# microsoft/rl-offline-simulation

Measured on AMD Instinct MI355X. Metric: simulated steps/sec (node), 10M logged transitions x 4096 rollouts, higher is better.
Workload: dtype f64

## Files before the change

### rl-offline-simulation_amd/csrc/offsim_hip.hip

```cpp
#include <hip/hip_fp16.h>
#include <hip/hip_runtime.h>
#include <mutex>
#include <stdint.h>
#include <stdio.h>
#include <stdlib.h>
#include <string.h>
#include <time.h>

#include "offsim.h"
#include "discount.hpp"
#include "pcg64_dev.hpp"
#include "philox_dev.hpp"

extern "C" int offsim_lds_order_ok(void);
#include "shuffle_wave.hpp"
#include "shuffle_chunk.hpp"

using namespace offsim;

static thread_local char g_err[512] = "";

static int fail(int code, const char *fmt, const char *detail = "") {
    snprintf(g_err, sizeof(g_err), fmt, detail);
    return code;
// ... 62 lines not shown
        if (s < n_slots) seg_off[s] = carry + inc - v;
        carry += __shfl(inc, WAVE - 1);
    }
    if (lane == 0) seg_off[n_slots] = carry;
}
__global__ void k_group_scatter(const int32_t *__restrict__ slot, int64_t N, int32_t n_slots,
                                const uint32_t *__restrict__ hist, const uint32_t *__restrict__ seg_off,
                                int32_t *__restrict__ order) {
    extern __shared__ uint32_t lds_pos_raw[];
    volatile uint32_t *lds_pos = lds_pos_raw;
    const uint32_t *h = hist + (int64_t)blockIdx.x * n_slots;
    for (int s = threadIdx.x; s < n_slots; s += WAVE) lds_pos[s] = seg_off[s] + h[s];
    __syncthreads();
    int lane = threadIdx.x;
    int64_t base = (int64_t)blockIdx.x * GRP_CHUNK;
    for (int i = 0; i < GRP_CHUNK; i += WAVE) {
        int64_t row = base + i + lane;
        bool valid = row < N;
        int32_t key = valid ? slot[row] : -1;
        uint64_t todo = __ballot(valid);
        uint32_t dst = 0;
        while (todo) {
            int leader = __ffsll((unsigned long long)todo) - 1;
            int32_t k = __shfl(key, leader);
            uint64_t same = __ballot(valid && key == k);
            if (valid && key == k) {
                uint32_t before = __popcll(same & ((1ull << lane) - 1ull));
                dst = lds_pos[k] + before;
            }
            __builtin_amdgcn_s_waitcnt(0xc07f);
            if (lane == leader) lds_pos[k] += __popcll(same);
            todo &= ~same;
        }
        if (valid) order[dst] = (int32_t)row;
    }
}

extern "C" int64_t offsim_group_scratch_bytes(int64_t N, int32_t n_slots) {
    int64_t n_chunks = (N + GRP_CHUNK - 1) / GRP_CHUNK;
    if (n_chunks < 1) n_chunks = 1;
    return (n_chunks * n_slots + n_slots) * (int64_t)sizeof(uint32_t) + 256;
}

extern "C" int offsim_group_by_state(const int32_t *slot, int64_t N, int32_t n_slots, uint32_t *seg_off, int32_t *order,
                                     void *scratch, void *stream) {
    if (N < 0 || n_slots <= 0 || !seg_off || !scratch) return fail(OFFSIM_EINVAL, "group_by_state: bad argument%s");
    if ((int64_t)n_slots * 4 > 64 * 1024) return fail(OFFSIM_EUNSUPPORTED, "group_by_state: more than 16384 states%s");
    if (N >= (1ll << 31)) return fail(OFFSIM_EUNSUPPORTED, "group_by_state: N >= 2^31%s");
    hipStream_t st = (hipStream_t)stream;
    int64_t n_chunks = (N + GRP_CHUNK - 1) / GRP_CHUNK;
    uint32_t *hist = (uint32_t *)scratch;
    uint32_t *totals = hist + (n_chunks > 0 ? n_chunks : 1) * n_slots;
    if (n_chunks == 0) {
        HIP_TRY(hipMemsetAsync(seg_off, 0, sizeof(uint32_t) * (n_slots + 1), st));
        return OFFSIM_OK;
    }
    size_t lds = sizeof(uint32_t) * n_slots;
    hipLaunchKernelGGL(k_group_hist, dim3((unsigned)n_chunks), dim3(256), lds, st, slot, N, n_slots, hist);
    LAUNCH_CHECK();
    hipLaunchKernelGGL(k_group_scan_chunks, dim3((n_slots + 63) / 64), dim3(64), 0, st, hist, n_chunks, n_slots, totals);
    LAUNCH_CHECK();
    hipLaunchKernelGGL(k_group_scan_slots, dim3(1), dim3(WAVE), 0, st, totals, n_slots, seg_off);
    LAUNCH_CHECK();
    hipLaunchKernelGGL(k_group_scatter, dim3((unsigned)n_chunks), dim3(WAVE), lds, st, slot, N, n_slots, hist, seg_off, order);
    LAUNCH_CHECK();
    return OFFSIM_OK;
}

template <typename T>
__global__ void k_gather_elem(const T *__restrict__ src, const int32_t *__restrict__ order, int64_t N, T *__restrict__ dst) {
    int64_t g = (int64_t)blockIdx.x * blockDim.x + threadIdx.x;
    if (g < N) dst[g] = src[order[g]];
}
template <typename W>
__global__ void k_gather_words(const W *__restrict__ src, const int32_t *__restrict__ order, int64_t N, int32_t words, W *__restrict__ dst) {
    int64_t i = (int64_t)blockIdx.x * blockDim.x + threadIdx.x;
    if (i >= N * words) return;
    int64_t g = i / words;
    int32_t w = (int32_t)(i - g * words);
    dst[i] = src[(int64_t)order[g] * words + w];
}
extern "C" int offsim_gather_rows(const void *src, const int32_t *order, int64_t N, int32_t row_bytes, void *dst, void *stream) {
    if (N < 0 || row_bytes <= 0) return fail(OFFSIM_EINVAL, "gather_rows: bad argument%s");
    if (N == 0) return OFFSIM_OK;
    hipStream_t st = (hipStream_t)stream;
    unsigned nb = (unsigned)((N + 255) / 256);
    if (row_bytes == 1) hipLaunchKernelGGL(k_gather_elem<uint8_t>, dim3(nb), dim3(256), 0, st, (const uint8_t *)src, order, N, (uint8_t *)dst);
    else if (row_bytes == 2) hipLaunchKernelGGL(k_gather_elem<uint16_t>, dim3(nb), dim3(256), 0, st, (const uint16_t *)src, order, N, (uint16_t *)dst);
    else if (row_bytes == 4) hipLaunchKernelGGL(k_gather_elem<uint32_t>, dim3(nb), dim3(256), 0, st, (const uint32_t *)src, order, N, (uint32_t *)dst);
    else if (row_bytes == 8) hipLaunchKernelGGL(k_gather_elem<uint64_t>, dim3(nb), dim3(256), 0, st, (const uint64_t *)src, order, N, (uint64_t *)dst);
    else {
        const int32_t wb = row_bytes % 4 == 0 ? 4 : row_bytes % 2 == 0 ? 2 : 1, words = row_bytes / wb;
        unsigned nbw = (unsigned)((N * words + 255) / 256);
        if (wb == 4) hipLaunchKernelGGL(k_gather_words<uint32_t>, dim3(nbw), dim3(256), 0, st, (const uint32_t *)src, order, N, words, (uint32_t *)dst);
        else if (wb == 2) hipLaunchKernelGGL(k_gather_words<uint16_t>, dim3(nbw), dim3(256), 0, st, (const uint16_t *)src, order, N, words, (uint16_t *)dst);
        else hipLaunchKernelGGL(k_gather_words<uint8_t>, dim3(nbw), dim3(256), 0, st, (const uint8_t *)src, order, N, words, (uint8_t *)dst);
    }
    LAUNCH_CHECK();
    return OFFSIM_OK;
}

__global__ void k_seed_streams(const uint64_t *__restrict__ seeds, int32_t R, uint64_t *__restrict__ out) {
    int r = blockIdx.x * blockDim.x + threadIdx.x;
    if (r >= R) return;
    PcgInit p = pcg_seed(seeds[r]);
    out[4 * r + 0] = p.state.hi;
    out[4 * r + 1] = p.state.lo;
    out[4 * r + 2] = p.inc.hi;
    out[4 * r + 3] = p.inc.lo;
}
extern "C" int offsim_seed_streams(const uint64_t *seeds, int32_t R, uint64_t *rng_out, void *stream) {
    if (R < 0 || !seeds || !rng_out) return fail(OFFSIM_EINVAL, "seed_streams: bad argument%s");
    if (R == 0) return OFFSIM_OK;
    hipLaunchKernelGGL(k_seed_streams, dim3((R + 255) / 256), dim3(256), 0, (hipStream_t)stream, seeds, R, rng_out);
    LAUNCH_CHECK();
    return OFFSIM_OK;
}

static hipError_t allow_big_lds_fn(const void *fn, int bytes) {
    struct Seen {
        const void *fn;
        int max_bytes;
        uint64_t devs;
    };
    static thread_local Seen seen[64];
    static thread_local int n_seen = 0;
    int dev = 0;
    hipError_t e = hipGetDevice(&dev);
    if (e != hipSuccess) return e;
    Seen *hit = nullptr;
    for (int i = 0; i < n_seen; i++)
        if (seen[i].fn == fn) hit = &seen[i];
    if (hit && dev < 64 && bytes <= hit->max_bytes && ((hit->devs >> dev) & 1ull)) return hipSuccess;
    const int want = hit && hit->max_bytes > bytes ? hit->max_bytes : bytes;
    e = hipFuncSetAttribute(fn, hipFuncAttributeMaxDynamicSharedMemorySize, want);
    if (e != hipSuccess) return e;
    if (!hit && n_seen < 64) {
        hit = &seen[n_seen++];
        hit->fn = fn;
        hit->max_bytes = 0;
        hit->devs = 0;
    }
    if (hit) {
        if (want > hit->max_bytes) {
            hit->max_bytes = want;
            hit->devs = 0;
        }
        if (dev < 64) hit->devs |= 1ull << dev;
    }
    return hipSuccess;
}
#define allow_big_lds(kernel, bytes) allow_big_lds_fn((const void *)(kernel), (bytes))

static int lds_order_ok_on(void *stream);
static int launch_shuffle(const offsim_table *t, const uint64_t *seeds, int32_t n_perm, uint32_t *perm_out, uint32_t *init_perm_out,
                          const uint32_t *dig32, uint32_t *dig_out, uint16_t *loc_out, hipStream_t st, bool big_segments_elsewhere = false) {
    const uint32_t max_seg = t->max_seg > 0 ? (uint32_t)(t->max_seg > 0xffffffffll ? 0xffffffffll : t->max_seg) : 0xffffffffu;
    const uint32_t min_seg = t->min_seg > 0 ? (uint32_t)(t->min_seg > 0xffffffffll ? 0xffffffffll : t->min_seg) : 1u;
    const uint32_t n0 = (uint32_t)(t->N0 > 0xffffffffll ? 0xffffffffll : t->N0);
    const int64_t n_blocks = (int64_t)(t->n_slots + 1) * n_perm;
    if (n_blocks > 0x7fffffffll) return fail(OFFSIM_EUNSUPPORTED, "shuffle_queues: too many chains%s");
    HIP_TRY(allow_big_lds((k_shuffle_wave<true, SHUF_SQ_BIG>), 160 * 1024));
    HIP_TRY(allow_big_lds((k_shuffle_wave<true, SHUF_SQ_SMALL>), 160 * 1024));
    static const bool no_xchg = getenv("OFFSIM_SHUFFLE_XCHG") && atoi(getenv("OFFSIM_SHUFFLE_XCHG")) == 0;
    const int okv = lds_order_ok_on(st);
    if (okv < 0) return okv;
    const uint32_t a_xchg = (okv == 1 && !no_xchg) ? 1u : 0u;
    if (!big_segments_elsewhere && (max_seg > SHUF_CAP16 || n0 > SHUF_CAP16)) {
        hipLaunchKernelGGL((k_shuffle_wave<false, SHUF_SQ_SMALL>), dim3((unsigned)n_blocks), dim3(256), shuf_fixed_lds_bytes(SHUF_SQ_SMALL), st, t->seg_off,
                           t->n_slots, t->N, t->N0, seeds, n_perm, perm_out, init_perm_out, SHUF_CAP16, 0xffffffffu, dig32, dig_out, loc_out, 0u);
        LAUNCH_CHECK();
    }
    static const uint32_t bounds[] = {SHUF_CAP16, 32768u, 8192u, 2048u, 0u};
    for (int k = 0; k < 4; k++) {
        const uint32_t hi = bounds[k], lo = bounds[k + 1];
        const bool seg_in = min_seg <= hi && max_seg > lo, init_in = n0 > lo && n0 <= hi;
        if (!seg_in && !init_in) continue;
        uint32_t need = 0;
        if (seg_in) need = max_seg < hi ? max_seg : hi;
        if (init_in && n0 > need) need = n0;
        const uint32_t sq = k == 0 ? SHUF_SQ_BIG : SHUF_SQ_SMALL;
        const size_t lds16 = shuf_fixed_lds_bytes(sq) + (((size_t)need * 2 + 15) & ~(size_t)15) + 16;
        if (k == 0 && dig_out) {
#define SHUF_LAUNCH(SQ, TOP, STOP, LDSB)                                                                                              \
    do {                                                                                                                              \
        HIP_TRY(allow_big_lds((k_shuffle_wave<true, SQ, TOP, STOP>), 160 * 1024));                                                     \
        hipLaunchKernelGGL((k_shuffle_wave<true, SQ, TOP, STOP>), dim3((unsigned)n_blocks), dim3(256), (LDSB), st, t->seg_off, t->n_slots, \
                           t->N, t->N0, seeds, n_perm, perm_out, init_perm_out, lo, hi, dig32, dig_out, loc_out, a_xchg);             \
        LAUNCH_CHECK();                                                                                                               \
    } while (0)
#define SHUF_TAILB(TOP) (shuf_fixed_lds_bytes(SHUF_SQ_SMALL) + (size_t)(TOP) * 2 + 16)
#ifdef SHUF_PROF
            const int prof_launches = getenv("OFFSIM_SHUFFLE_PROF_LAUNCHES") ? atoi(getenv("OFFSIM_SHUFFLE_PROF_LAUNCHES")) : 3;
#else
            const int prof_launches = 3;
#endif
            SHUF_LAUNCH(SHUF_SQ_BIG, 0, SHUF_CUT_HI, lds16);
            if (prof_launches >= 2) SHUF_LAUNCH(SHUF_SQ_SMALL, SHUF_CUT_HI, SHUF_CUT_LO, SHUF_TAILB(SHUF_CUT_HI));
            if (prof_launches >= 3) SHUF_LAUNCH(SHUF_SQ_SMALL, SHUF_CUT_LO, 1, SHUF_TAILB(SHUF_CUT_LO));
#undef SHUF_LAUNCH
#undef SHUF_TAILB
            if (init_in)
                hipLaunchKernelGGL((k_shuffle_wave<true, SHUF_SQ_BIG>), dim3((unsigned)n_perm), dim3(256), lds16, st, t->seg_off, t->n_slots, t->N,
                                   t->N0, seeds, n_perm, perm_out, init_perm_out, lo, hi, dig32, nullptr, nullptr, a_xchg);
        } else if (k == 0)
            hipLaunchKernelGGL((k_shuffle_wave<true, SHUF_SQ_BIG>), dim3((unsigned)n_blocks), dim3(256), lds16, st, t->seg_off, t->n_slots, t->N, t->N0,
                               seeds, n_perm, perm_out, init_perm_out, lo, hi, dig32, dig_out, loc_out, a_xchg);
        else
            hipLaunchKernelGGL((k_shuffle_wave<true, SHUF_SQ_SMALL>), dim3((unsigned)n_blocks), dim3(256), lds16, st, t->seg_off, t->n_slots, t->N, t->N0,
                               seeds, n_perm, perm_out, init_perm_out, lo, hi, dig32, dig_out, loc_out, a_xchg);
        LAUNCH_CHECK();
    }
    return OFFSIM_OK;
}

__global__ void k_fault_exchange(int32_t *out) { *out = atomicExch(&offsim::g_async_fault, 0); }

extern "C" int offsim_async_faults(void) {
    static int32_t *slot[64] = {nullptr};
    static std::mutex mu;
    std::lock_guard<std::mutex> hold(mu);
    int dev = 0;
    if (hipGetDevice(&dev) != hipSuccess || dev < 0 || dev >= 64) return fail(OFFSIM_EHIP, "async_faults: no device%s");
    if (!slot[dev] && hipMalloc((void **)&slot[dev], sizeof(int32_t)) != hipSuccess) return fail(OFFSIM_EHIP, "async_faults: allocation failed%s");
    hipLaunchKernelGGL(k_fault_exchange, dim3(1), dim3(1), 0, (hipStream_t)0, slot[dev]);
    if (hipGetLastError() != hipSuccess) return fail(OFFSIM_EHIP, "async_faults: launch failed%s");
    int32_t v = 0;
    if (hipMemcpy(&v, slot[dev], sizeof(v), hipMemcpyDeviceToHost) != hipSuccess) return fail(OFFSIM_EHIP, "async_faults: read failed%s");
    return v;
}

extern "C" int offsim_shuffle_queues(const offsim_table *t, const uint64_t *seeds, int32_t n_perm, uint32_t *perm_out,
                                     uint32_t *init_perm_out, void *stream) {
    if (!t || !seeds || n_perm < 0 || !perm_out || !init_perm_out) return fail(OFFSIM_EINVAL, "shuffle_queues: bad argument%s");
    if (n_perm == 0) return OFFSIM_OK;
    return launch_shuffle(t, seeds, n_perm, perm_out, init_perm_out, nullptr, nullptr, nullptr, (hipStream_t)stream);
}

__global__ void __launch_bounds__(256) k_big_keys(const uint32_t *__restrict__ seg_off, int64_t N, const uint32_t *__restrict__ dig32,
                                                  uint32_t *__restrict__ dig_out, uint16_t *__restrict__ loc_out, uint32_t r0) {
    const uint32_t s = blockIdx.y, r = r0 + blockIdx.z;
    const uint32_t beg = seg_off[s], len = seg_off[s + 1] - beg;
    if (len <= SHUF_CAP16) return;
    for (uint32_t k = blockIdx.x * 1024u + threadIdx.x; k < len && k < (blockIdx.x + 1u) * 1024u; k += 256u) {
        const int64_t p = (int64_t)r * N + beg + k;
        const uint32_t row = dig_out[p], loc = row - beg, h = loc >> 16;
        dig_out[p] = dig32[row] | ((h & 3u) << 8) | ((h >> 2) << 11);
        loc_out[p] = (uint16_t)loc;
    }
}

#define SHC_HEADER_BYTES 4096
static uint32_t shc_cb() {
    static const int v = getenv("OFFSIM_SHUFFLE_CHUNK") ? atoi(getenv("OFFSIM_SHUFFLE_CHUNK")) : 0;
    return v == 16384 ? 16384u : v == 8192 ? 8192u : v == 2048 ? 2048u : 4096u;
}
static uint32_t shc_longest(const offsim_table *t) {
    const int64_t a = t->max_seg > (int64_t)SHUF_CAP16 ? t->max_seg : 0, b = t->N0 > (int64_t)SHUF_CAP16 ? t->N0 : 0;
    return (uint32_t)(a > b ? a : b);
}
static int64_t shc_block_words(const offsim_table *t, uint32_t *msg_cap_out, int64_t *lc_words_out = nullptr, bool plain = false) {
    const uint32_t n = shc_longest(t), cb = shc_cb();
    const uint64_t msg = shc_pool_entries(n, cb), rep = (uint64_t)((n + cb - 1u) / cb) * cb;
    if (msg_cap_out) *msg_cap_out = (uint32_t)msg;
    if (lc_words_out) *lc_words_out = plain ? 0 : (int64_t)((n + 3u) / 4u);
    if (plain) return (int64_t)(msg + rep);
    return (int64_t)(msg + (msg + 1u) / 2u + rep + (n + 3u) / 4u);
}
extern "C" int64_t offsim_shuffle_workspace_bytes(const offsim_table *t, int32_t n_blocks) {
    if (!t || n_blocks < 1 || shc_longest(t) == 0 || t->max_seg > (1ll << 23) || t->N0 > (1ll << 23)) return 0;
    return SHC_HEADER_BYTES + (int64_t)n_blocks * shc_block_words(t, nullptr) * 8;
}

struct ShcPlan {
    int64_t n_wg = 0, words = 0, lc_words = 0;
    uint32_t msg_cap = 0, kcap = 0, lds_b = 0;
};
static ShcPlan shc_plan(const offsim_table *t, void *workspace, int64_t workspace_bytes, bool plain) {
    ShcPlan p;
    if (shc_longest(t) == 0 || t->max_seg > (1ll << 23) || t->N0 > (1ll << 23) || !workspace || ((uintptr_t)workspace & 7u) != 0) return p;
    if (t->n_slots + 1 > (SHC_HEADER_BYTES / 4 - 64)) return p;
    p.words = shc_block_words(t, &p.msg_cap, &p.lc_words, plain);
    p.n_wg = (workspace_bytes - SHC_HEADER_BYTES) / (p.words * 8);
    int dev = 0, cus = 256;
    if (hipGetDevice(&dev) == hipSuccess) (void)hipDeviceGetAttribute(&cus, hipDeviceAttributeMultiprocessorCount, dev);
    p.kcap = (shc_longest(t) + shc_cb() - 1u) / shc_cb();
#define SHC_LDSB(PL)                                                                                                                    \
    (shc_cb() == 16384u ? shc_lds_bytes<16384u, 2048u, 1024u, PL>(p.kcap) : shc_cb() == 4096u ? shc_lds_bytes<4096u, 1024u, 512u, PL>(p.kcap) \
     : shc_cb() == 2048u ? shc_lds_bytes<2048u, 1024u, 512u, PL>(p.kcap) : shc_lds_bytes<8192u, 1024u, 512u, PL>(p.kcap))
    p.lds_b = plain ? SHC_LDSB(true) : SHC_LDSB(false);
#undef SHC_LDSB
    const int64_t per_cu = (160 * 1024) / (int64_t)((p.lds_b + 1023u) & ~1023u);
    p.n_wg = p.n_wg > cus * per_cu ? cus * per_cu : p.n_wg;
    if (p.n_wg < 1) p.n_wg = 0;
    return p;
}
static int shc_launch(const ShcPlan &p, const offsim_table *t, const uint64_t *seeds, int32_t n_perm, const uint32_t *dig32, uint32_t *dig_out,
                      void *loc_out, uint32_t *init_perm_out, uint32_t *perm_out, void *workspace, hipStream_t st, uint32_t loc_bits = 16u,
                      uint32_t chains_above = SHUF_CAP16) {
    { const int okv = lds_order_ok_on(st); if (okv < 0) return okv; if (okv == 0) return fail(OFFSIM_EUNSUPPORTED, "chunked shuffle: this device's LDS does not serve same-address lanes of one instruction in lane order (offsim_lds_order_ok): lend no workspace -- the in-place shuffle does not need it%s"); }
    uint32_t *hdr = (uint32_t *)workspace;
    hipLaunchKernelGGL(k_chunk_worklist, dim3(1), dim3(256), 0, st, t->seg_off, t->n_slots, (uint32_t)(t->N0 > 0xffffffffll ? 0xffffffffll : t->N0), chains_above,
                       hdr + 64, hdr + 1, hdr);
    LAUNCH_CHECK();
#define SHC_LAUNCH_(CB, RG, SQ, PL)                                                                                                     \
    do {                                                                                                                                \
        HIP_TRY(allow_big_lds((k_shuffle_chunked<CB, RG, SQ, PL>), 160 * 1024));                                                         \
        hipLaunchKernelGGL((k_shuffle_chunked<CB, RG, SQ, PL>), dim3((unsigned)p.n_wg), dim3(256), p.lds_b, st, t->seg_off, t->N, seeds, n_perm,  \
                           hdr + 64, hdr + 1, hdr, (uint64_t *)((char *)workspace + SHC_HEADER_BYTES), p.words, p.msg_cap, p.kcap, dig32,   \
                           dig_out, loc_out, t->n_slots, t->N0, init_perm_out, perm_out, p.lc_words, loc_bits);                         \
    } while (0)
#define SHC_LAUNCH(CB, RG, SQ)                                                                                                          \
    do {                                                                                                                                \
        if (perm_out) SHC_LAUNCH_(CB, RG, SQ, true);                                                                                    \
        else SHC_LAUNCH_(CB, RG, SQ, false);                                                                                            \
    } while (0)
    if (shc_cb() == 16384u) SHC_LAUNCH(16384u, 2048u, 1024u);
    else if (shc_cb() == 4096u) SHC_LAUNCH(4096u, 1024u, 512u);
    else if (shc_cb() == 2048u) SHC_LAUNCH(2048u, 1024u, 512u);
    else SHC_LAUNCH(8192u, 1024u, 512u);
#undef SHC_LAUNCH
#undef SHC_LAUNCH_
    LAUNCH_CHECK();
    return OFFSIM_OK;
}

extern "C" int offsim_shuffle_queues_ws(const offsim_table *t, const uint64_t *seeds, int32_t n_perm, uint32_t *perm_out, uint32_t *init_perm_out,
                                        void *workspace, int64_t workspace_bytes, void *stream) {
    if (!t || !seeds || n_perm < 0 || !perm_out || !init_perm_out) return fail(OFFSIM_EINVAL, "shuffle_queues: bad argument%s");
    if (n_perm == 0) return OFFSIM_OK;
    const ShcPlan p = t->max_seg > 0 ? shc_plan(t, workspace, workspace_bytes, true) : ShcPlan();
    int rc = launch_shuffle(t, seeds, n_perm, perm_out, init_perm_out, nullptr, nullptr, nullptr, (hipStream_t)stream, p.n_wg >= 1);
    if (rc || p.n_wg < 1) return rc;
    return shc_launch(p, t, seeds, n_perm, nullptr, nullptr, nullptr, init_perm_out, perm_out, workspace, (hipStream_t)stream);
}

extern "C" int offsim_shuffle_queues_keys_ws(const offsim_table *t, const uint64_t *seeds, int32_t n_perm, const uint32_t *dig32, int32_t format,
                                             uint32_t *dig_out, void *loc_out, uint32_t *init_perm_out, void *workspace, int64_t workspace_bytes,
                                             void *stream) {
    if (!t || !seeds || n_perm < 0 || !init_perm_out || (t->N > 0 && (!dig32 || !dig_out || !loc_out)))
        return fail(OFFSIM_EINVAL, "shuffle_queues_keys: bad argument%s");
    if (format != OFFSIM_STREAMS_A && format != OFFSIM_STREAMS_B && format != OFFSIM_STREAMS_C) return fail(OFFSIM_EINVAL, "shuffle_queues_keys: bad format%s");
    if (t->max_seg <= 0 && t->N > 0) return fail(OFFSIM_EINVAL, "shuffle_queues_keys: offsim_table.max_seg must be set%s");
    const bool big = t->max_seg > (int64_t)SHUF_CAP16;
    if (format == OFFSIM_STREAMS_C) {
        if (t->max_seg > (1ll << 17) || t->n_slots > 255 || t->N0 > (1ll << 23))
            return fail(OFFSIM_EUNSUPPORTED, "shuffle_queues_keys: format C holds 2^17 rows per state, 255 states%s");
        if (n_perm == 0 || t->N == 0) return OFFSIM_OK;
        offsim_table tc = *t;
        if (tc.max_seg <= (int64_t)SHUF_CAP16) tc.max_seg = (int64_t)SHUF_CAP16 + 1;
        const ShcPlan pc = shc_plan(&tc, workspace, workspace_bytes, false);
        if (pc.n_wg < 1) return fail(OFFSIM_EUNSUPPORTED, "shuffle_queues_keys: format C needs a workspace (offsim_shuffle_workspace_bytes)%s");
        return shc_launch(pc, &tc, seeds, n_perm, dig32, dig_out, loc_out, init_perm_out, nullptr, workspace, (hipStream_t)stream, 8u, 0u);
    }
// ... 1657 lines not shown
```

### rl-offline-simulation_amd/csrc/shuffle_wave.hpp

```cpp
#pragma once
#include <type_traits>
#include <hip/hip_runtime.h>
#include <stdint.h>

#include "pcg64_dev.hpp"

namespace offsim {

#define SHUF_RG 2048u
#ifndef SHUF_CUT_HI
#define SHUF_CUT_HI 16384u
#endif
#ifndef SHUF_CUT_LO
#define SHUF_CUT_LO 4096u
#endif
#define SHUF_SQ_BIG 4096u
#define SHUF_SQ_SMALL 1024u
#define SHUF_CAP16 65536u
enum { SH_GEN0 = 0, SH_GEN1 = 1, SH_CPUB = 2, SH_FILL = 3, SH_TAIL = 4, SH_DONE = 5, SH_ATOP = 6, SH_EM0 = 7, SH_EM1 = 8, SH_CSTOP = 9,
       SH_ABORT = 10 };
__device__ int32_t g_async_fault = 0;
#define SHUF_SPIN_LIMIT (1u << 20)
__device__ __noinline__ void shuf_bound_check(volatile __attribute__((address_space(3))) uint32_t *ctrl, uint32_t polls) {
    if (polls > SHUF_SPIN_LIMIT) ctrl[SH_ABORT] = 1u;
    if (ctrl[SH_ABORT]) {
        if ((threadIdx.x & 63u) == 0u) atomicOr(&g_async_fault, OFFSIM_FAULT_SHUFFLE);
        __builtin_amdgcn_endpgm();
    }
}
__device__ __forceinline__ void shuf_bound(volatile __attribute__((address_space(3))) uint32_t *ctrl, uint32_t &polls) {
#ifndef SHUF_NO_BOUND
    if (__builtin_expect((++polls & 1023u) == 0u, 0)) shuf_bound_check(ctrl, polls);
#endif
}
#define SHUF_CH 512u

typedef __attribute__((address_space(3))) volatile uint32_t lds_vu32;
typedef __attribute__((address_space(3))) volatile uint16_t lds_vu16;
typedef __attribute__((address_space(3))) volatile uint64_t lds_vu64;

__device__ __forceinline__ uint32_t sh_rfl(uint32_t v) { return (uint32_t)__builtin_amdgcn_readfirstlane(v); }
__device__ __forceinline__ uint32_t sh_ld(lds_vu32 *p) { return sh_rfl(*p); }
__device__ __forceinline__ void sh_st(lds_vu32 *p, uint32_t v) { *p = v; }
__device__ __forceinline__ uint64_t sh_lowmask(uint32_t k) { return k >= 64u ? ~0ull : ((1ull << k) - 1ull); }
__device__ __forceinline__ uint32_t sh_ff1(uint64_t m) { return (uint32_t)__ffsll((unsigned long long)m) - 1u; }
__device__ __forceinline__ int sh_rank(uint64_t m) {
    return (int)__builtin_amdgcn_mbcnt_hi((uint32_t)(m >> 32), __builtin_amdgcn_mbcnt_lo((uint32_t)m, 0u));
}

constexpr uint32_t shuf_fixed_lds_bytes(uint32_t sq) { return 4u * (16u + SHUF_RG + sq + 64u + 64u); }

template <bool LDS16, uint32_t SHUF_SQ, uint32_t TOP = 0, uint32_t STOP = 1>
__global__ void __launch_bounds__(256)
    k_shuffle_wave(const uint32_t *__restrict__ seg_off, int32_t n_slots, int64_t N, int64_t N0, const uint64_t *__restrict__ seeds,
                   int32_t n_perm, uint32_t *__restrict__ perm, uint32_t *__restrict__ init_perm, uint32_t n_lo, uint32_t n_hi,
                   const uint32_t *__restrict__ dig32, uint32_t *__restrict__ dig_out, uint16_t *__restrict__ loc_out, uint32_t a_xchg) {
    extern __shared__ __align__(16) unsigned char lds_raw[];
    lds_vu32 *ctrl = (lds_vu32 *)lds_raw;
    lds_vu32 *ring = ctrl + 16;
    lds_vu32 *jq = ring + SHUF_RG;
    lds_vu32 *win = jq + SHUF_SQ + 64u;
    lds_vu16 *x16 = (lds_vu16 *)(win + 64u);
    const int wave = __builtin_amdgcn_readfirstlane(threadIdx.x >> 6), lane = threadIdx.x & 63;

    const int32_t s_idx = (int32_t)(blockIdx.x / (uint32_t)n_perm);
    const int32_t r = (int32_t)(blockIdx.x - (uint32_t)s_idx * (uint32_t)n_perm);
    const int32_t s = s_idx == 0 ? n_slots : s_idx - 1;
    uint32_t n, base_val;
    uint32_t *xg;
    if (s < n_slots) {
        const uint32_t b = seg_off[s];
        n = seg_off[s + 1] - b;
        xg = perm + (int64_t)r * N + b;
        base_val = b;
    } else {
        n = (uint32_t)N0;
        xg = init_perm + (int64_t)r * N0;
        base_val = 0;
    }
    if (n == 0) return;
    if (n <= n_lo || (LDS16 && n > n_hi)) return;
    volatile uint32_t *x32 = (volatile uint32_t *)xg;
    constexpr bool FROM_STREAM = TOP != 0u, CUT = STOP > 1u;
    static_assert(!(FROM_STREAM || CUT) || LDS16, "the cut form is for LDS-resident keyed chains");
    static_assert((TOP & (TOP - 1u)) == 0u && (STOP & (STOP - 1u)) == 0u && (TOP == 0u || TOP > STOP), "cuts are powers of two");
    if ((FROM_STREAM || CUT) && (dig_out == nullptr || s >= n_slots)) return;
    const uint32_t n_rows = n;
    if (FROM_STREAM) n = TOP;
    const uint32_t stop_i = STOP;

    const bool keyed = LDS16 && dig_out != nullptr && s < n_slots;
    const uint32_t *dsrc = keyed ? dig32 + base_val : nullptr;
    uint32_t *dg = keyed ? dig_out + (int64_t)r * N + base_val : nullptr;
    uint16_t *lc = keyed ? loc_out + (int64_t)r * N + base_val : nullptr;
    const uint32_t n_chunks = (n + SHUF_CH - 1u) / SHUF_CH;
    auto emit_chunk = [&](uint32_t ch) {
        lds_vu32 *xw = (lds_vu32 *)x16;
        const uint32_t pairs = (n + 1u) >> 1, k0 = ch * (SHUF_CH / 2u) + (uint32_t)lane;
        uint32_t two[4], d0[4], d1[4];
#pragma unroll
        for (int u = 0; u < 4; u++) {
            const uint32_t k = k0 + 64u * (uint32_t)u;
            two[u] = k < pairs ? xw[k] : 0u;
        }
        if (CUT && ch < STOP / SHUF_CH) {
#pragma unroll
            for (int u = 0; u < 4; u++) {
                const uint32_t k = k0 + 64u * (uint32_t)u;
                lc[2u * k] = (uint16_t)(two[u] & 0xffffu);
                lc[2u * k + 1u] = (uint16_t)(two[u] >> 16);
            }
            return;
        }
#pragma unroll
        for (int u = 0; u < 4; u++) {
            const uint32_t i1 = two[u] >> 16;
            d0[u] = dsrc[two[u] & 0xffffu];
            d1[u] = dsrc[i1 < n_rows ? i1 : 0u];
        }
#pragma unroll
        for (int u = 0; u < 4; u++) {
            const uint32_t k = k0 + 64u * (uint32_t)u;
            if (k < pairs) {
                dg[2u * k] = d0[u];
                lc[2u * k] = (uint16_t)(two[u] & 0xffffu);
                if (2u * k + 1u < n) {
                    dg[2u * k + 1u] = d1[u];
                    lc[2u * k + 1u] = (uint16_t)(two[u] >> 16);
                }
            }
        }
    };

    if (threadIdx.x < 16u) ctrl[threadIdx.x] = threadIdx.x == SH_ATOP ? n - 1u : (threadIdx.x == SH_EM0 || threadIdx.x == SH_EM1) ? n_chunks : 0u;
    if (threadIdx.x < 64u) win[threadIdx.x] = 0;
    uint32_t c_start = 0;
    if (FROM_STREAM) {
        c_start = dg[0];
        for (uint32_t k = threadIdx.x; k < TOP; k += 256u) x16[k] = lc[k];
    } else if (LDS16) {
        __attribute__((address_space(3))) uint32_t *xw = (__attribute__((address_space(3))) uint32_t *)x16;
        for (uint32_t k = threadIdx.x; 2u * k < n; k += 256u) xw[k] = ((2u * k + 1u) << 16) | (2u * k);
    } else {
        for (uint32_t k = threadIdx.x; k < n; k += 256u) xg[k] = base_val + k;
    }
    __syncthreads();

#ifdef SHUF_PROF
    uint64_t pf_wait = 0, pf_w0 = 0, pf_extra = 0;
    const uint64_t pf_begin = __builtin_amdgcn_s_memtime();
#define SPW0() pf_w0 = __builtin_amdgcn_s_memtime()
#define SPW1() pf_wait += __builtin_amdgcn_s_memtime() - pf_w0
#define SPX1() pf_extra += __builtin_amdgcn_s_memtime() - pf_w0
#else
#define SPW0()
#define SPW1()
#define SPX1()
#endif
    if (n >= 2) {
        if (wave == 0 || wave == 3) {
            const uint32_t g = wave == 0 ? 0u : 1u;
            const PcgInit p = pcg_seed(seeds[r]);
            const Jump j128 = pcg_jump(p.inc, 128);
            U128 st = pcg_apply(pcg_jump(p.inc, (uint64_t)(c_start >> 1) + 64ull * g + (uint64_t)lane + 1), p.state);
            uint32_t blk = g, done_blocks = 0, cpub = 0;
            int32_t em_next = (int32_t)n_chunks - 1 - (int32_t)(((n_chunks - 1u) & 1u) != g);
            for (;;) {
                bool stop = false;
                SPW0();
                uint32_t polls = 0;
                while ((blk + 1u) * 128u - cpub > SHUF_RG) {
                    shuf_bound(ctrl, polls);
                    if (sh_ld(ctrl + SH_DONE)) {
                        stop = true;
                        break;
                    }
                    if (keyed && em_next >= 0 && sh_ld(ctrl + SH_ATOP) < SHUF_CH * (uint32_t)em_next) {
#ifdef SHUF_PROF
                        const uint64_t e0 = __builtin_amdgcn_s_memtime();
                        emit_chunk((uint32_t)em_next);
                        pf_extra += __builtin_amdgcn_s_memtime() - e0;
#else
                        emit_chunk((uint32_t)em_next);
#endif
                        sh_st(ctrl + (g ? SH_EM1 : SH_EM0), (uint32_t)em_next);
                        em_next -= 2;
                    } else {
                        __builtin_amdgcn_s_sleep(1);
                    }
                    cpub = sh_ld(ctrl + SH_CPUB);
                }
                SPW1();
                if (stop) break;
                const uint64_t o = pcg_output(st);
                st = pcg_apply(j128, st);
                const uint32_t idx = (blk * 128u + 2u * (uint32_t)lane) & (SHUF_RG - 1u);
                *(lds_vu64 *)(ring + idx) = o;
                blk += 2u;
                done_blocks++;
                sh_st(ctrl + (g ? SH_GEN1 : SH_GEN0), done_blocks);
            }
        } else if (wave == 1) {
            uint32_t i = n - 1u, c = c_start & 1u, avail = 0, fill = 0, tail = 0;
            uint32_t mask = 0xffffffffu >> __builtin_clz(i);
            int lowpow = (int)((mask >> 1) + 1u);
            auto wait_draws = [&](uint32_t upto) {
                if (__builtin_expect(upto <= avail, 1)) return;
                const bool waited = upto > avail;
                if (waited) SPW0();
                uint32_t polls = 0;
                while (upto > avail) {
                    const uint64_t gg = *(lds_vu64 *)(ctrl + SH_GEN0);
                    const uint32_t g0 = sh_rfl((uint32_t)gg), g1 = sh_rfl((uint32_t)(gg >> 32));
                    avail = 128u * (g0 <= g1 ? 2u * g0 : 2u * g1 + 1u);
                    if (upto > avail) {
                        shuf_bound(ctrl, polls);
                        __builtin_amdgcn_s_sleep(1);
                    }
                }
                if (waited) SPW1();
            };
            auto wait_room = [&](uint32_t upto) {
                if (__builtin_expect(upto - tail <= SHUF_SQ, 1)) return;
                const bool waited = upto - tail > SHUF_SQ;
                if (waited) SPW0();
                uint32_t polls = 0;
                while (upto - tail > SHUF_SQ) {
                    tail = sh_ld(ctrl + SH_TAIL);
                    if (upto - tail > SHUF_SQ) {
                        shuf_bound(ctrl, polls);
                        __builtin_amdgcn_s_sleep(1);
                    }
                }
                if (waited) SPX1();
            };
            auto settle = [&](uint64_t &bal, int &rk, uint32_t v, uint32_t ib) {
                uint64_t f = bal & __ballot((int)v > (int)ib - rk);
                while (f) {
                    bal &= ~(1ull << sh_ff1(f));
                    rk = sh_rank(bal);
                    f = bal & __ballot((int)v > (int)ib - rk);
                }
            };
            wait_draws(c + 128u);
            uint32_t ra = ring[c + (uint32_t)lane], rb = ring[c + 64u + (uint32_t)lane], rc = 0, rd = 0;
#ifndef SHUF_C_PAIRS
#define SHUF_C_PAIRS 2
#endif
            auto iter = [&](auto SEL, const bool publish) __attribute__((always_inline)) {
                constexpr bool S = decltype(SEL)::value;
                const uint32_t r1 = S ? rc : ra, r2 = S ? rd : rb;
                wait_draws(c + 256u);
                uint32_t p1 = ring[(c + 128u + (uint32_t)lane) & (SHUF_RG - 1u)];
                uint32_t p2 = ring[(c + 192u + (uint32_t)lane) & (SHUF_RG - 1u)];
                const uint32_t v1 = r1 & mask, v2 = r2 & mask;
                uint64_t bal1 = __ballot(v1 <= i);
                uint32_t n1 = (uint32_t)__popcll(bal1);
                uint32_t i2 = i - n1;
                uint64_t bal2 = __ballot((int)v2 <= (int)i2);
                int rk1 = sh_rank(bal1), rk2 = sh_rank(bal2);
                const uint64_t f1 = bal1 & __ballot((int)v1 > (int)i - rk1), f2 = bal2 & __ballot((int)v2 > (int)i2 - rk2);
                if (__builtin_expect((f1 | f2) != 0ull, 0)) {
                    if (f1) {
                        settle(bal1, rk1, v1, i);
                        n1 = (uint32_t)__popcll(bal1);
                        i2 = i - n1;
                        bal2 = __ballot((int)v2 <= (int)i2);
                        rk2 = sh_rank(bal2);
                    }
                    if ((bal2 & __ballot((int)v2 > (int)i2 - rk2)) != 0ull) settle(bal2, rk2, v2, i2);
                }
                const uint32_t n2 = (uint32_t)__popcll(bal2);
                const int i_new = (int)i2 - (int)n2;
                if (__builtin_expect(i_new >= lowpow, 1)) {
                    wait_room(fill + n1 + n2);
                    uint32_t a1, a2;
                    asm("v_cndmask_b32_e64 %0, %1, %2, %3" : "=v"(a1) : "v"(SHUF_SQ + (uint32_t)lane), "v"((fill + (uint32_t)rk1) & (SHUF_SQ - 1u)), "s"(bal1));
                    asm("v_cndmask_b32_e64 %0, %1, %2, %3" : "=v"(a2) : "v"(SHUF_SQ + (uint32_t)lane), "v"((fill + n1 + (uint32_t)rk2) & (SHUF_SQ - 1u)), "s"(bal2));
                    jq[a1] = v1;
                    jq[a2] = v2;
                    fill += n1 + n2;
                    sh_st(ctrl + SH_FILL, fill);
                    i = (uint32_t)i_new;
                    c += 128u;
                } else {
                    const uint64_t lowm = __ballot((int)i - rk1 < lowpow);
                    const uint64_t below = (lowm & (0ull - lowm)) - 1ull;
                    const uint64_t acc = bal1 & below;
                    const uint32_t na = (uint32_t)__popcll(acc);
                    wait_room(fill + na);
                    jq[((acc >> lane) & 1ull) ? ((fill + (uint32_t)rk1) & (SHUF_SQ - 1u)) : SHUF_SQ + (uint32_t)lane] = v1;
                    fill += na;
                    sh_st(ctrl + SH_FILL, fill);
                    i -= na;
                    c += (uint32_t)__popcll(below);
                    if ((int)i < lowpow && i >= 1u) {
                        mask = 0xffffffffu >> __builtin_clz(i);
                        lowpow = (int)((mask >> 1) + 1u);
                    }
                    wait_draws(c + 128u);
                    p1 = ring[(c + (uint32_t)lane) & (SHUF_RG - 1u)];
                    p2 = ring[(c + 64u + (uint32_t)lane) & (SHUF_RG - 1u)];
                }
                if (S) {
                    ra = p1;
                    rb = p2;
                } else {
                    rc = p1;
                    rd = p2;
                }
                if (publish) sh_st(ctrl + SH_CPUB, c);
            };
#if SHUF_C_PAIRS == 1
            while (i >= stop_i) {
                iter(std::false_type{}, true);
                ra = rc;
                rb = rd;
            }
#else
            while (i >= stop_i) {
                iter(std::false_type{}, false);
                if (__builtin_expect(i < stop_i, 0)) break;
                iter(std::true_type{}, true);
            }
            sh_st(ctrl + SH_CPUB, c);
#endif
            if (CUT) sh_st(ctrl + SH_CSTOP, (c_start & ~1u) + c);
            sh_st(ctrl + SH_DONE, 1u);
        } else {
            uint32_t i_top = n - 1u, done = 0, fill = 0;
            auto xrd = [&](uint32_t k) -> uint32_t { return LDS16 ? (uint32_t)x16[k] : x32[k]; };
            auto xwr = [&](uint32_t k, uint32_t val) {
                if (LDS16) x16[k] = (uint16_t)val;
                else x32[k] = val;
            };
            auto piecewise = [&](uint32_t cnt, uint32_t i_first, uint32_t il, uint32_t v, uint32_t b, uint32_t tg, uint64_t confl, uint64_t F) {
                const bool in = (uint32_t)lane < cnt;
                if (in) xwr(v, b);
                uint64_t cuts = 0;
                while (confl) {
                    cuts |= 1ull << (i_first - sh_rfl((uint32_t)__builtin_amdgcn_readlane((int)v, (int)sh_ff1(confl))));
                    confl &= confl - 1ull;
                }
                if (F) {
                    const bool lost = tg != (uint32_t)lane;
                    if (lost) win[tg] = 1u;
                    const uint32_t w = win[(uint32_t)lane];
                    if (lost) win[tg] = 0u;
                    const uint64_t D = F | __ballot(w != 0u);
                    cuts |= D & (D - 1ull);
                }
                const uint32_t pid = in ? (uint32_t)sh_rank(cuts) + (uint32_t)((cuts >> lane) & 1ull) : 0xffffffffu;
                const uint32_t n_pieces = (uint32_t)__popcll(cuts & sh_lowmask(cnt) & ~1ull) + 1u;
// ... 134 lines not shown
                "v_mov_b32_e32 %[d], %[it]\n\t"                                                                              \
                "ds_write_b32 %[ctrl], %[m] offset:16\n\t"                                                      \
                "ds_write_b32 %[ctrl], %[d] offset:24\n\t"
                asm volatile(
                    "s_and_b32 s20, %[done], %[sqm]\n\t"
                    "v_lshl_add_u32 %[ja], s20, 2, %[jql]\n\t"
                    "ds_read_b32 %[v], %[ja]\n\t"
                    "v_lshl_add_u32 %[ja], %[il], 1, %[x16a]\n\t"
                    "ds_read_u16 %[a], %[ja]\n\t"
                    "s_waitcnt lgkmcnt(0)\n\t"
                    "s_branch 82f\n\t"
#if SHUF_A_GROUPS >= 4
                    SHUF_AX_GROUP("80", "82", "3", "84f", "")
                    SHUF_AX_GROUP("84", "85", "1", "86f", "")
                    SHUF_AX_GROUP("86", "87", "1", "81f", "")
#else
                    SHUF_AX_GROUP("80", "82", "3", "81f", "")
#endif
                    SHUF_AX_GROUP("81", "83", "1", "80b", SHUF_AX_PUBLISH)
                    "91:\n\t"
                    "s_mov_b32 %[code], 1\n\t"
                    "s_branch 99f\n\t"
                    "92:\n\t"
                    "s_mov_b32 %[code], 0\n\t"
                    "s_branch 94f\n\t"
                    "93:\n\t"
                    "s_mov_b32 %[code], 2\n\t"
                    "94:\n\t"
                    "s_waitcnt lgkmcnt(0)\n\t"
                    "s_nop 0\n\t"
                    "v_lshrrev_b32_e32 %[old], %[sh], %[old]\n\t"
                    "ds_write_b16 %[wa], %[old]\n\t"
                    "99:\n\t"
                    "s_waitcnt lgkmcnt(0)"
                    : [it] "+s"(i_top), [done] "+s"(done), [il] "+v"(il_cur), [v] "+v"(v_cur), [a] "+v"(a_cur), [code] "=&s"(code), [sh] "=&v"(t_sh),
                      [ad] "=&v"(t_ad), [m] "=&v"(t_m), [d] "=&v"(t_d), [old] "=&v"(t_old), [wa] "=&v"(t_wa), [ja] "=&v"(t_ja)
                    : [fill] "s"(fill), [lo64] "s"(64u + lo), [sqm] "s"(SHUF_SQ - 1u), [x16a] "v"(x16_a), [jql] "v"(jq_lane), [ffff] "v"(0xffffu),
                      [ctrl] "v"(ctrl_a)
                    : "vcc", "scc", "memory", "s20", "s21", "s22", "s23");
                static_assert(SH_TAIL == 4 && SH_ATOP == 6, "the immediates of the applier's loop");
#undef SHUF_AX_GROUP
#undef SHUF_AX_PUBLISH
                return code;
            };
#ifndef SHUF_A_ASM
#define SHUF_A_ASM 1
#endif
            if (LDS16 && a_xchg && SHUF_A_ASM) {
                while (i_top >= 64u + lo) {
                    if (__builtin_expect(fill - done < 64u, 0)) {
                        SPW0();
                        uint32_t polls = 0;
                        while (fill - done < 64u) {
                            fill = sh_ld(ctrl + SH_FILL);
                            if (fill - done < 64u) {
                                shuf_bound(ctrl, polls);
                                __builtin_amdgcn_s_sleep(1);
                            }
                        }
                        SPW1();
                    }
                    const uint32_t code = run_x();
                    if (code == 1u) {
                        SPW0();
                        const uint32_t i_first = i_top, il = i_first - (uint32_t)lane, v = v_cur;
                        done += 64u;
                        i_top -= 64u;
                        const uint64_t confl = __ballot(v < il) & __ballot(v > i_top);
                        const uint32_t b = (uint32_t)x16[v];
                        x16[v] = (uint16_t)lane;
                        const uint32_t tg = (uint32_t)x16[v];
                        piecewise(64u, i_first, il, v, b, tg, confl, __ballot(tg != (uint32_t)lane));
                        SPX1();
                    }
                    sh_st(ctrl + SH_TAIL, done);
                    sh_st(ctrl + SH_ATOP, i_top);
                }
            } else if (LDS16 && a_xchg) {
                if (i_top >= 64u + lo) for (;;) {
                    group_x(false);
                    if (__builtin_expect(i_top < 64u + lo, 0)) break;
                    group_x(true);
                    if (__builtin_expect(i_top < 64u + lo, 0)) break;
                }
            } else
            if (i_top >= 64u + lo) for (;;) {
#if SHUF_A_GROUPS >= 4
                group(false);
                if (__builtin_expect(i_top < 64u + lo, 0)) break;
                group(false);
                if (__builtin_expect(i_top < 64u + lo, 0)) break;
#endif
#if SHUF_A_GROUPS >= 2
                group(false);
                if (__builtin_expect(i_top < 64u + lo, 0)) break;
#endif
                group(true);
                if (__builtin_expect(i_top < 64u + lo, 0)) break;
            }
            sh_st(ctrl + SH_TAIL, done);
            sh_st(ctrl + SH_ATOP, i_top);
            if (i_top > lo) {
                const uint32_t cnt = i_top - lo;
                uint32_t polls = 0;
                while (fill - done < cnt) {
                    fill = sh_ld(ctrl + SH_FILL);
                    if (fill - done < cnt) {
                        shuf_bound(ctrl, polls);
                        __builtin_amdgcn_s_sleep(1);
                    }
                }
                const uint32_t v = jq[(done + (uint32_t)lane) & (SHUF_SQ - 1u)];
                const uint32_t il = i_top - (uint32_t)lane;
                const bool in = (uint32_t)lane < cnt;
                const uint64_t confl = __ballot(in && v < il && v > lo);
                uint32_t b = 0, tg = (uint32_t)lane;
                if (in) {
                    b = xrd(v);
                    xwr(v, (uint32_t)lane);
                    tg = xrd(v);
                }
                piecewise(cnt, i_top, il, v, b, tg, confl, __ballot(tg != (uint32_t)lane));
            }
        }
    }
#ifdef SHUF_PROF
    const uint64_t pf_end = __builtin_amdgcn_s_memtime();
#endif
    __syncthreads();
    if (LDS16) {
        __attribute__((address_space(3))) const uint32_t *xw = (__attribute__((address_space(3))) const uint32_t *)x16;
        if (keyed) {
            const uint32_t em0 = ctrl[SH_EM0], em1 = ctrl[SH_EM1];
            for (uint32_t ch = (uint32_t)wave; ch < n_chunks; ch += 4u)
                if (ch < ((ch & 1u) ? em1 : em0)) emit_chunk(ch);
        } else {
            for (uint32_t k = threadIdx.x; 2u * k < n; k += 256u) {
                const uint32_t two = xw[k];
                xg[2u * k] = base_val + (two & 0xffffu);
                if (2u * k + 1u < n) xg[2u * k + 1u] = base_val + (two >> 16);
            }
        }
    }
    if (CUT) {
        __syncthreads();
        if (threadIdx.x == 0) dg[0] = ctrl[SH_CSTOP];
    }
#ifdef SHUF_PROF
    __syncthreads();
    if (keyed && lane == 0 && n >= 64u) {
        dg[3 * wave + 0] = (uint32_t)((pf_end - pf_begin) >> 6);
        dg[3 * wave + 1] = (uint32_t)(pf_wait >> 6);
        dg[3 * wave + 2] = (uint32_t)(pf_extra >> 6);
        if (wave == 0) dg[12] = (uint32_t)((__builtin_amdgcn_s_memtime() - pf_begin) >> 6);
    }
#endif
}

}
```

Before: 15.66 billion.

## Split shuffle into configurable cut stages and vectorize stream-to-LDS fill

Replaces the fixed three-launch shuffle split (cuts at 16384 and 4096) with a compile-time list of cuts, defaulting to 32768, 8192 and 2048, so the shuffle runs as four staged launches. Each stage is launched through a recursive template. The per-stage refill of LDS from the previous stage's 16-bit stream now uses 16-byte vector loads, with alignbyte fixups for odd-aligned sources, instead of scalar 16-bit copies. The aim is to shrink per-stage LDS footprint and reload cost, at the price of an extra launch and an extra stream round trip. Profiling counters are also extended.

New measurement: 16.15 billion, median of 6. +3.2%, better.

```diff
diff --git a/rl-offline-simulation_amd/csrc/offsim_hip.hip b/rl-offline-simulation_amd/csrc/offsim_hip.hip
--- a/rl-offline-simulation_amd/csrc/offsim_hip.hip
+++ b/rl-offline-simulation_amd/csrc/offsim_hip.hip
@@ -238,6 +238,24 @@
 }
 #define allow_big_lds(kernel, bytes) allow_big_lds_fn((const void *)(kernel), (bytes))
 
+template <int K>
+static int shuf_launch_cuts(int n_launches, size_t lds_top, unsigned n_blocks, hipStream_t st, const offsim_table *t, const uint64_t *seeds, int32_t n_perm,
+                            uint32_t *perm_out, uint32_t *init_perm_out, uint32_t lo, uint32_t hi, const uint32_t *dig32, uint32_t *dig_out,
+                            uint16_t *loc_out, uint32_t a_xchg) {
+    constexpr uint32_t TOP = K == 0 ? 0u : shuf_cuts[K > 0 ? K - 1 : 0], STOP = K == shuf_n_cuts ? 1u : shuf_cuts[K < shuf_n_cuts ? K : 0];
+    constexpr uint32_t SQ = K == 0 ? SHUF_SQ_BIG : SHUF_SQ_SMALL;
+    if (K >= n_launches) return OFFSIM_OK;
+    const size_t ldsb = K == 0 ? lds_top : shuf_fixed_lds_bytes(SQ) + (size_t)TOP * 2 + 16;
+    HIP_TRY(allow_big_lds((k_shuffle_wave<true, SQ, TOP, STOP>), 160 * 1024));
+    hipLaunchKernelGGL((k_shuffle_wave<true, SQ, TOP, STOP>), dim3(n_blocks), dim3(256), ldsb, st, t->seg_off, t->n_slots, t->N, t->N0, seeds, n_perm,
+                       perm_out, init_perm_out, lo, hi, dig32, dig_out, loc_out, a_xchg);
+    LAUNCH_CHECK();
+    if constexpr (K < shuf_n_cuts)
+        return shuf_launch_cuts<K + 1>(n_launches, lds_top, n_blocks, st, t, seeds, n_perm, perm_out, init_perm_out, lo, hi, dig32, dig_out, loc_out, a_xchg);
+    else
+        return OFFSIM_OK;
+}
+
 static int lds_order_ok_on(void *stream);
 static int launch_shuffle(const offsim_table *t, const uint64_t *seeds, int32_t n_perm, uint32_t *perm_out, uint32_t *init_perm_out,
                           const uint32_t *dig32, uint32_t *dig_out, uint16_t *loc_out, hipStream_t st, bool big_segments_elsewhere = false) {
@@ -268,24 +286,14 @@
         const uint32_t sq = k == 0 ? SHUF_SQ_BIG : SHUF_SQ_SMALL;
         const size_t lds16 = shuf_fixed_lds_bytes(sq) + (((size_t)need * 2 + 15) & ~(size_t)15) + 16;
         if (k == 0 && dig_out) {
-#define SHUF_LAUNCH(SQ, TOP, STOP, LDSB)                                                                                              \
-    do {                                                                                                                              \
-        HIP_TRY(allow_big_lds((k_shuffle_wave<true, SQ, TOP, STOP>), 160 * 1024));                                                     \
-        hipLaunchKernelGGL((k_shuffle_wave<true, SQ, TOP, STOP>), dim3((unsigned)n_blocks), dim3(256), (LDSB), st, t->seg_off, t->n_slots, \
-                           t->N, t->N0, seeds, n_perm, perm_out, init_perm_out, lo, hi, dig32, dig_out, loc_out, a_xchg);             \
-        LAUNCH_CHECK();                                                                                                               \
-    } while (0)
-#define SHUF_TAILB(TOP) (shuf_fixed_lds_bytes(SHUF_SQ_SMALL) + (size_t)(TOP) * 2 + 16)
 #ifdef SHUF_PROF
-            const int prof_launches = getenv("OFFSIM_SHUFFLE_PROF_LAUNCHES") ? atoi(getenv("OFFSIM_SHUFFLE_PROF_LAUNCHES")) : 3;
+            const int prof_launches = getenv("OFFSIM_SHUFFLE_PROF_LAUNCHES") ? atoi(getenv("OFFSIM_SHUFFLE_PROF_LAUNCHES")) : shuf_n_cuts + 1;
 #else
-            const int prof_launches = 3;
+            const int prof_launches = shuf_n_cuts + 1;
 #endif
-            SHUF_LAUNCH(SHUF_SQ_BIG, 0, SHUF_CUT_HI, lds16);
-            if (prof_launches >= 2) SHUF_LAUNCH(SHUF_SQ_SMALL, SHUF_CUT_HI, SHUF_CUT_LO, SHUF_TAILB(SHUF_CUT_HI));
-            if (prof_launches >= 3) SHUF_LAUNCH(SHUF_SQ_SMALL, SHUF_CUT_LO, 1, SHUF_TAILB(SHUF_CUT_LO));
-#undef SHUF_LAUNCH
-#undef SHUF_TAILB
+            const int rc = shuf_launch_cuts<0>(prof_launches, lds16, (unsigned)n_blocks, st, t, seeds, n_perm, perm_out, init_perm_out, lo, hi, dig32, dig_out,
+                                               loc_out, a_xchg);
+            if (rc != OFFSIM_OK) return rc;
             if (init_in)
                 hipLaunchKernelGGL((k_shuffle_wave<true, SHUF_SQ_BIG>), dim3((unsigned)n_perm), dim3(256), lds16, st, t->seg_off, t->n_slots, t->N,
                                    t->N0, seeds, n_perm, perm_out, init_perm_out, lo, hi, dig32, nullptr, nullptr, a_xchg);
diff --git a/rl-offline-simulation_amd/csrc/shuffle_wave.hpp b/rl-offline-simulation_amd/csrc/shuffle_wave.hpp
--- a/rl-offline-simulation_amd/csrc/shuffle_wave.hpp
+++ b/rl-offline-simulation_amd/csrc/shuffle_wave.hpp
@@ -8,12 +8,17 @@
 namespace offsim {
 
 #define SHUF_RG 2048u
-#ifndef SHUF_CUT_HI
-#define SHUF_CUT_HI 16384u
-#endif
-#ifndef SHUF_CUT_LO
-#define SHUF_CUT_LO 4096u
-#endif
+#ifndef SHUF_CUT_LIST
+#define SHUF_CUT_LIST 32768u, 8192u, 2048u
+#endif
+constexpr uint32_t shuf_cuts[] = {SHUF_CUT_LIST};
+constexpr int shuf_n_cuts = (int)(sizeof(shuf_cuts) / sizeof(shuf_cuts[0]));
+constexpr bool shuf_cuts_ok() {
+    for (int k = 0; k < shuf_n_cuts; k++)
+        if ((shuf_cuts[k] & (shuf_cuts[k] - 1u)) != 0u || shuf_cuts[k] < 1024u || (k == 0 ? shuf_cuts[k] > 32768u : shuf_cuts[k] >= shuf_cuts[k - 1])) return false;
+    return true;
+}
+static_assert(shuf_cuts_ok(), "SHUF_CUT_LIST: descending powers of two, 32768 at most, 1024 at least");
 #define SHUF_SQ_BIG 4096u
 #define SHUF_SQ_SMALL 1024u
 #define SHUF_CAP16 65536u
@@ -48,6 +53,54 @@
     return (int)__builtin_amdgcn_mbcnt_hi((uint32_t)(m >> 32), __builtin_amdgcn_mbcnt_lo((uint32_t)m, 0u));
 }
 
+template <uint32_t TOP>
+__device__ __forceinline__ void shuf_fill_from_stream(lds_vu16 *x16, const uint16_t *lc) {
+    typedef uint32_t u32x4_a4 __attribute__((ext_vector_type(4), aligned(4)));
+    typedef uint32_t u32x4 __attribute__((ext_vector_type(4)));
+    constexpr uint32_t VEC = TOP / 8u, J = VEC ? (VEC + 255u) / 256u : 1u;
+    static_assert(TOP % 8u == 0u, "the fill moves 16 bytes at a time");
+    const bool odd = (((uintptr_t)lc >> 1) & 1u) != 0u;
+    const uint32_t *src = (const uint32_t *)(lc - (odd ? 1 : 0));
+    __attribute__((address_space(3))) u32x4 *dst = (__attribute__((address_space(3))) u32x4 *)x16;
+    u32x4 w[J];
+    if (odd) {
+        uint32_t e[J];
+#pragma unroll
+        for (uint32_t j = 0; j < J; j++) {
+            const uint32_t q = threadIdx.x + 256u * j;
+            if (VEC % 256u == 0u || q < VEC) {
+                w[j] = *(const u32x4_a4 *)(src + 4u * q);
+                e[j] = src[4u * q + 4u];
+            }
+        }
+        __builtin_amdgcn_sched_barrier(0);
+#pragma unroll
+        for (uint32_t j = 0; j < J; j++) {
+            const uint32_t q = threadIdx.x + 256u * j;
+            if (VEC % 256u == 0u || q < VEC) {
+                u32x4 o;
+                o.x = __builtin_amdgcn_alignbyte(w[j].y, w[j].x, 2u);
+                o.y = __builtin_amdgcn_alignbyte(w[j].z, w[j].y, 2u);
+                o.z = __builtin_amdgcn_alignbyte(w[j].w, w[j].z, 2u);
+                o.w = __builtin_amdgcn_alignbyte(e[j], w[j].w, 2u);
+                dst[q] = o;
+            }
+        }
+    } else {
+#pragma unroll
+        for (uint32_t j = 0; j < J; j++) {
+            const uint32_t q = threadIdx.x + 256u * j;
+            if (VEC % 256u == 0u || q < VEC) w[j] = *(const u32x4_a4 *)(src + 4u * q);
+        }
+        __builtin_amdgcn_sched_barrier(0);
+#pragma unroll
+        for (uint32_t j = 0; j < J; j++) {
+            const uint32_t q = threadIdx.x + 256u * j;
+            if (VEC % 256u == 0u || q < VEC) dst[q] = w[j];
+        }
+    }
+}
+
 constexpr uint32_t shuf_fixed_lds_bytes(uint32_t sq) { return 4u * (16u + SHUF_RG + sq + 64u + 64u); }
 
 template <bool LDS16, uint32_t SHUF_SQ, uint32_t TOP = 0, uint32_t STOP = 1>
@@ -61,6 +114,9 @@
     lds_vu32 *jq = ring + SHUF_RG;
     lds_vu32 *win = jq + SHUF_SQ + 64u;
     lds_vu16 *x16 = (lds_vu16 *)(win + 64u);
+#ifdef SHUF_PROF
+    const uint64_t pf_entry = __builtin_amdgcn_s_memtime();
+#endif
     const int wave = __builtin_amdgcn_readfirstlane(threadIdx.x >> 6), lane = threadIdx.x & 63;
 
     const int32_t s_idx = (int32_t)(blockIdx.x / (uint32_t)n_perm);
@@ -137,7 +193,7 @@
     uint32_t c_start = 0;
     if (FROM_STREAM) {
         c_start = dg[0];
-        for (uint32_t k = threadIdx.x; k < TOP; k += 256u) x16[k] = lc[k];
+        shuf_fill_from_stream<TOP>(x16, lc);
     } else if (LDS16) {
         __attribute__((address_space(3))) uint32_t *xw = (__attribute__((address_space(3))) uint32_t *)x16;
         for (uint32_t k = threadIdx.x; 2u * k < n; k += 256u) xw[k] = ((2u * k + 1u) << 16) | (2u * k);
@@ -147,7 +203,7 @@
     __syncthreads();
 
 #ifdef SHUF_PROF
-    uint64_t pf_wait = 0, pf_w0 = 0, pf_extra = 0;
+    uint64_t pf_wait = 0, pf_w0 = 0, pf_extra = 0, pf_g_first = 0;
     const uint64_t pf_begin = __builtin_amdgcn_s_memtime();
 #define SPW0() pf_w0 = __builtin_amdgcn_s_memtime()
 #define SPW1() pf_wait += __builtin_amdgcn_s_memtime() - pf_w0
@@ -199,6 +255,9 @@
                 blk += 2u;
                 done_blocks++;
                 sh_st(ctrl + (g ? SH_GEN1 : SH_GEN0), done_blocks);
+#ifdef SHUF_PROF
+                if (done_blocks == 1u) pf_g_first = __builtin_amdgcn_s_memtime() - pf_begin;
+#endif
             }
         } else if (wave == 1) {
             uint32_t i = n - 1u, c = c_start & 1u, avail = 0, fill = 0, tail = 0;
@@ -639,7 +698,12 @@
         dg[3 * wave + 0] = (uint32_t)((pf_end - pf_begin) >> 6);
         dg[3 * wave + 1] = (uint32_t)(pf_wait >> 6);
         dg[3 * wave + 2] = (uint32_t)(pf_extra >> 6);
-        if (wave == 0) dg[12] = (uint32_t)((__builtin_amdgcn_s_memtime() - pf_begin) >> 6);
+        if (wave == 0) {
+            dg[12] = (uint32_t)((__builtin_amdgcn_s_memtime() - pf_begin) >> 6);
+            dg[13] = (uint32_t)((pf_begin - pf_entry) >> 6);
+            dg[15] = (uint32_t)(pf_g_first >> 6);
+        }
+        if (wave == 1) dg[14] = (uint32_t)((__builtin_amdgcn_s_memtime() - pf_end) >> 6);
     }
 #endif
 }
```
